# SamGalanakis/FlowCompare

Hardware: AMD Instinct MI355X
Metric: nats/sec (forward log-prob) on 4096-pt coloured pairs (higher is better)
Workload: dtype fp16x2 split (fp32-equivalent operands, f32 accumulate) / f32; 1 GPU; c2_dgcnn_attn_spline: batch 16 scenes/GPU x 4096 target + 4096 context points, 115 flow layers (RationalQuadraticSplineCoupling), embedder DGCNNembedder; global_batch=16, parallelism=scene-sharded x1, no data-path collective

## Files before the change

### flowcompare_amd/csrc/mlprows.hip

```cpp
#include "common.h"
#include "activations.h"
#include "mlprows.h"
#include <type_traits>
#include <cstdio>

namespace fc {

typedef float floatx16 __attribute__((ext_vector_type(16)));
typedef _Float16 f16x8 __attribute__((ext_vector_type(8)));
typedef __attribute__((address_space(3))) char mr_lds_char;
typedef const __attribute__((address_space(1))) char mr_glb_char;

constexpr int MR_KSTG = 8;
constexpr int MR_STAGE = MR_KSTG * 2 * 1024;
constexpr int MR_R = 8, MR_D = 6;
constexpr int MR_PPW = MR_KSTG * 2 / 4;
constexpr int MR_NWAIT = (MR_D - 1) * MR_PPW;
constexpr int MR_BIAS_OFF = MR_R * MR_STAGE;
constexpr int MR_LDS = MR_BIAS_OFF + 2 * MR_HID * 4;

__device__ __forceinline__ void mr_swap32(unsigned& a, unsigned& b) {
    asm("s_nop 1\n\tv_permlane32_swap_b32 %0, %1\n\ts_nop 1" : "+v"(a), "+v"(b));
}
__device__ __forceinline__ unsigned mr_pack(_Float16 a, _Float16 b) {
    return (unsigned)__builtin_bit_cast(unsigned short, a) | ((unsigned)__builtin_bit_cast(unsigned short, b) << 16);
}
__device__ __forceinline__ float mr_lo(unsigned w) { return (float)__builtin_bit_cast(_Float16, (unsigned short)(w & 0xffffu)); }
__device__ __forceinline__ float mr_hi(unsigned w) { return (float)__builtin_bit_cast(_Float16, (unsigned short)(w >> 16)); }

typedef unsigned mr_u4 __attribute__((ext_vector_type(4)));
typedef float mr_f4 __attribute__((ext_vector_type(4)));
__device__ __forceinline__ mr_u4 mr_gload16(const char* ptr) {
    mr_u4 r;
    asm volatile("global_load_dwordx4 %0, %1, off" : "=v"(r) : "v"(ptr) : "memory");
    return r;
}
template <int N>
__device__ __forceinline__ void mr_wait_vm(mr_u4& a, mr_u4& b) {
    asm volatile("s_waitcnt vmcnt(%2)" : "+v"(a), "+v"(b) : "n"(N) : "memory");
}
__device__ __forceinline__ mr_f4 mr_lds_read16(unsigned addr) {
    mr_f4 r;
    asm volatile("ds_read_b128 %0, %1" : "=v"(r) : "v"(addr) : "memory");
    return r;
}
__device__ __forceinline__ void mr_wait_lgkm(mr_f4& a, mr_f4& b, mr_f4& c, mr_f4& d) {
    asm volatile("s_waitcnt lgkmcnt(0)" : "+v"(a), "+v"(b), "+v"(c), "+v"(d) : : "memory");
}

template <int ACT>
__device__ __forceinline__ float mr_act(float v) {
    if constexpr (ACT == FC_ACT_GELU) return fc_gelu(v);
    else if constexpr (ACT == FC_ACT_RELU) return v > 0.f ? v : 0.f;
    else if constexpr (ACT == FC_ACT_ELU) return v > 0.f ? v : expm1f(v);
    else if constexpr (ACT == FC_ACT_LRELU02) return v > 0.f ? v : 0.2f * v;
    else return v;
}

#define MR_STAMP(K_)                                                                                                  \
    if (STAMPS && p.stamps && tid == 0 && (blockIdx.x == 0 || blockIdx.x == 300) && gcur < 256) {                               \
        __builtin_amdgcn_sched_barrier(0);                                                                            \
        p.stamps[((blockIdx.x ? 1 : 0) * 256 + (gcur - ((K_) > 2 ? 1 : 0))) * 8 + (K_)] = __builtin_amdgcn_s_memtime(); \
        __builtin_amdgcn_sched_barrier(0);                                                                            \
    }

template <int KS0, int ACT, bool STAMPS = false>
__global__ __launch_bounds__(256) __attribute__((amdgpu_waves_per_eu(1, 1)))
void mlp_rows_kernel(const MlpRowsParams p) {
    extern __shared__ char smc[];
    const int tid = threadIdx.x, lane = tid & 63, li = lane & 31, lh = lane >> 5;
    const int wave = __builtin_amdgcn_readfirstlane(tid >> 6);
    const int row = blockIdx.x * 128 + wave * 32 + li;
    const int row_in = row < p.rows_valid ? row : p.rows_valid - 1;
    const size_t band = (size_t)blockIdx.x * 4 + wave;
    const size_t band_bytes = (size_t)MR_HID / 16 * 2048;

    const char* ws_ptr = reinterpret_cast<const char*>(p.L[0].Wf) + (wave * MR_PPW) * 1024;
    const unsigned lane16 = lane * 16;
    int ws_left = (p.L[0].ks / MR_KSTG) * MR_NB, ws_layer = 0;
    unsigned ws_slot = 0;
    auto issue_piece = [&](auto i_tag) __attribute__((always_inline)) {
        constexpr int i = decltype(i_tag)::value;
        char* dst = smc + ws_slot * MR_STAGE + (wave * MR_PPW + i) * 1024;
        __builtin_amdgcn_global_load_lds((mr_glb_char*)(ws_ptr + i * 1024 + lane16), (mr_lds_char*)dst, 16, 0, 0);
        if constexpr (i == MR_PPW - 1) {
            ws_slot = (ws_slot + 1) % MR_R;
            if (--ws_left > 0) ws_ptr += MR_STAGE;
            else if (ws_layer + 1 < p.nlayers) {
                ++ws_layer;
                ws_ptr = reinterpret_cast<const char*>(p.L[ws_layer].Wf) + (wave * MR_PPW) * 1024;
                ws_left = (p.L[ws_layer].ks / MR_KSTG) * MR_NB;
            } else ws_left = 1;
        }
    };
    auto issue_stage = [&]() __attribute__((always_inline)) {
        issue_piece(std::integral_constant<int, 0>{}); issue_piece(std::integral_constant<int, 1>{});
        issue_piece(std::integral_constant<int, 2>{}); issue_piece(std::integral_constant<int, 3>{});
    };
    static_assert(MR_PPW == 4, "issue_stage / the slot table place four DMA pieces per wave and stage");
    auto stage_bias = [&](int l) __attribute__((always_inline)) {
        const MlpRowsLayer& L = p.L[l];
        if (wave < 2)
            __builtin_amdgcn_global_load_lds((mr_glb_char*)(reinterpret_cast<const char*>(L.bias) + wave * 1024 + lane * 16),
                                             (mr_lds_char*)(smc + MR_BIAS_OFF + wave * 1024), 16, 0, 0);
        else if (l == 0) {
            if (p.rowscal && L.colvec)
                __builtin_amdgcn_global_load_lds((mr_glb_char*)(reinterpret_cast<const char*>(L.colvec) + (wave - 2) * 1024 + lane * 16),
                                                 (mr_lds_char*)(smc + MR_BIAS_OFF + MR_HID * 4 + (wave - 2) * 1024), 16, 0, 0);
            else
                *reinterpret_cast<float4*>(smc + MR_BIAS_OFF + MR_HID * 4 + (wave - 2) * 1024 + lane * 16) = make_float4(0.f, 0.f, 0.f, 0.f);
        }
    };
    stage_bias(0);
#pragma unroll
    for (int i = 0; i < MR_D; ++i) issue_stage();
    unsigned gcur = 0;

    f16x8 xin[MR_HID / 16][2];
    float omax = 0.f;
    constexpr int MR_XA = 24;
    auto pin_xin = [&](int ks) __attribute__((always_inline)) {
#pragma unroll
        for (int s = 0; s < MR_HID / 16; ++s)
            if (s < MR_XA && s < ks) { asm volatile("" : "+a"(xin[s][0])); asm volatile("" : "+a"(xin[s][1])); }
    };

    {
        const int k0 = p.segk[0], k1 = k0 + p.segk[1], k2 = k1 + p.segk[2];
        float4 raw[KS0][2];
#pragma unroll
        for (int s = 0; s < KS0; ++s) {
            const int seg = s < k0 ? 0 : (s < k1 ? 1 : 2);
            const int sl = s - (seg == 0 ? 0 : (seg == 1 ? k0 : k1));
            const bool live = s < k2;
            const float* ptr = p.A[live ? seg : 0] + (size_t)row_in * p.lda[live ? seg : 0] + (live ? sl : 0) * 16 + 8 * lh;
            raw[s][0] = *reinterpret_cast<const float4*>(ptr);
            raw[s][1] = *reinterpret_cast<const float4*>(ptr + 4);
            if (!live) { raw[s][0] = make_float4(0.f, 0.f, 0.f, 0.f); raw[s][1] = raw[s][0]; }
        }
#pragma unroll
        for (int s = 0; s < KS0; ++s) {
            const float x[8] = {raw[s][0].x, raw[s][0].y, raw[s][0].z, raw[s][0].w, raw[s][1].x, raw[s][1].y, raw[s][1].z, raw[s][1].w};
#pragma unroll
            for (int e = 0; e < 8; ++e) {
                omax = fmaxf(omax, fabsf(x[e]));
                const _Float16 h = (_Float16)x[e];
                xin[s][0][e] = h;
                xin[s][1][e] = (_Float16)((x[e] - (float)h) * 2048.0f);
            }
        }
    }

    pin_xin(KS0);

    floatx16 accA, corrA, accB, corrB;
    mr_u4 resA_hi, resA_lo, resB_hi, resB_lo;
    mr_f4 bnext[4], cnext[4];
    unsigned outq[4][2][2];

    auto run_layer = [&](auto ks_tag, auto res_tag, auto first_tag, const int l) __attribute__((always_inline)) {
        constexpr int KS = decltype(ks_tag)::value;
        constexpr bool HAS_RES = decltype(res_tag)::value;
        constexpr bool FIRST = decltype(first_tag)::value;
        constexpr int NSB = KS / MR_KSTG;
        static_assert(!HAS_RES || NSB == 4, "only the 512 -> 512 hidden layers carry a residual");
        const MlpRowsLayer& L = p.L[l];
        const bool last = l + 1 == p.nlayers;
        const float sp1 = last ? p.out_s1 : 1.0f, sp2 = last ? p.out_s2 : 2048.0f;
        const char* resbase = HAS_RES ? reinterpret_cast<const char*>(p.hbuf[L.res]) + band * band_bytes + lane * 16 : nullptr;
        char* outbase = last ? reinterpret_cast<char*>(p.out16) + (size_t)row * (MR_HID / 16 * 64) + lh * 16
                             : reinterpret_cast<char*>(p.hbuf[L.out]) + band * band_bytes + lane * 16;
        const int out_ss = last ? 64 : 2048, out_ls = last ? 32 : 1024;
        const float rs = (FIRST && p.rowscal && L.colvec) ? p.rowscal[row_in] : 0.f;
        const unsigned bias_lds = (unsigned)(uintptr_t)(mr_lds_char*)smc + (unsigned)(MR_BIAS_OFF + 16 * lh);

        auto bias_fetch = [&](int nb) __attribute__((always_inline)) {
#pragma unroll
            for (int g = 0; g < 4; ++g) {
                bnext[g] = mr_lds_read16(bias_lds + (unsigned)(nb * 32 + 8 * g) * 4u);
                if constexpr (FIRST) cnext[g] = mr_lds_read16(bias_lds + (unsigned)(MR_HID + nb * 32 + 8 * g) * 4u);
            }
        };
        auto init_vec = [&]() __attribute__((always_inline)) -> floatx16 {
            mr_wait_lgkm(bnext[0], bnext[1], bnext[2], bnext[3]);
            if constexpr (FIRST) mr_wait_lgkm(cnext[0], cnext[1], cnext[2], cnext[3]);
            floatx16 b;
#pragma unroll
            for (int g = 0; g < 4; ++g)
#pragma unroll
                for (int t = 0; t < 4; ++t) {
                    b[4 * g + t] = bnext[g][t];
                    if constexpr (FIRST) b[4 * g + t] += rs * cnext[g][t];
                }
            return b;
        };

        float ev[2][4], eu[2][4], eg[2][4];
        auto epi_step = [&](const floatx16& pa, const floatx16& pc, auto g_tag, auto m_tag) __attribute__((always_inline)) {
            constexpr int g = decltype(g_tag)::value, m = decltype(m_tag)::value, pr = m / 12, hs = m % 12, Q = g & 1;
            static_assert(ACT == FC_ACT_GELU, "the interleaved epilogue is written for the exact-erf GELU of the shipped configurations");
            constexpr float C[12] = {7.953413483363647e-10f, -3.609737220244824e-08f, 7.156736501201522e-07f, -8.034509846766014e-06f, 5.399647488957271e-05f, -0.0001862359931692481f, -0.0002285758382640779f, 0.00727660721167922f, -0.05270823836326599f, -0.4591129422187805f, -1.151120901107788f, -0.9999995827674866f};
#define MR_PIN(X_) asm volatile("" : "+v"(X_))
#pragma unroll
            for (int tt = 0; tt < 2; ++tt) {
                const int t = 2 * pr + tt;
                if constexpr (hs == 0) {
                    float v = fmaf(pc[4 * g + t], 1.0f / 2048.0f, pa[4 * g + t]);
                    if constexpr (HAS_RES) {
                        const mr_u4& rh = g < 2 ? resA_hi : resB_hi;
                        const mr_u4& rl = g < 2 ? resA_lo : resB_lo;
                        const unsigned hw = (g & 1) ? (pr == 0 ? rh.z : rh.w) : (pr == 0 ? rh.x : rh.y);
                        const unsigned lw = (g & 1) ? (pr == 0 ? rl.z : rl.w) : (pr == 0 ? rl.x : rl.y);
                        v += tt ? limb_join<1>(hw, lw) : limb_join<0>(hw, lw);
                    }
                    MR_PIN(v);
                    ev[Q][t] = v;
                } else if constexpr (hs == 1) {
                    float u = fminf(fabsf(ev[Q][t]), 7.353910524340095f);
                    float gp = fmaf(C[0], u, C[1]);
                    MR_PIN(u); MR_PIN(gp);
                    eu[Q][t] = u; eg[Q][t] = gp;
                } else if constexpr (hs >= 2 && hs <= 4) {
                    float gp = eg[Q][t];
#pragma unroll
                    for (int c = 0; c < 3; ++c) gp = fmaf(gp, eu[Q][t], C[3 * hs - 4 + c]);
                    MR_PIN(gp);
                    eg[Q][t] = gp;
                } else if constexpr (hs == 5) {
                    float gp = fmaf(eg[Q][t], eu[Q][t], C[11]);
                    MR_PIN(gp);
                    eg[Q][t] = gp;
                } else if constexpr (hs == 6) {
                    float e = __builtin_amdgcn_exp2f(eg[Q][t]);
                    MR_PIN(e);
                    eg[Q][t] = e;
                } else if constexpr (hs == 7) {
                    float m;
                    asm("v_max_f32 %0, 0, %1" : "=v"(m) : "v"(ev[Q][t]));
                    float r = fmaf(-fabsf(ev[Q][t]), eg[Q][t], m);
                    MR_PIN(r);
                    ev[Q][t] = r;
                } else if constexpr (hs == 8) {
                    if (tt == 1) {
                        unsigned wh2, wl2;
                        limb_split2s(ev[Q][2 * pr], ev[Q][2 * pr + 1], sp1, sp2, wh2, wl2);
                        MR_PIN(wh2); MR_PIN(wl2);
                        outq[g][0][pr] = wh2;
                        outq[g][1][pr] = wl2;
                    }
                } else if constexpr (hs == 9) {
                    if (tt == 1) {
                        float om = fmaxf(omax, fmaxf(fabsf(ev[Q][2 * pr]), fabsf(ev[Q][2 * pr + 1])));
                        MR_PIN(om);
                        omax = om;
                    }
                }
            }
#undef MR_PIN
        };
        auto quarter = [&](const floatx16& pa, const floatx16& pc, auto g_tag) __attribute__((always_inline)) {
            auto go = [&](auto... ms) __attribute__((always_inline)) { (epi_step(pa, pc, g_tag, ms), ...); };
            go(std::integral_constant<int, 0>{}, std::integral_constant<int, 1>{}, std::integral_constant<int, 2>{}, std::integral_constant<int, 3>{},
               std::integral_constant<int, 4>{}, std::integral_constant<int, 5>{}, std::integral_constant<int, 6>{}, std::integral_constant<int, 7>{},
               std::integral_constant<int, 8>{}, std::integral_constant<int, 9>{}, std::integral_constant<int, 10>{}, std::integral_constant<int, 11>{},
               std::integral_constant<int, 12>{}, std::integral_constant<int, 13>{}, std::integral_constant<int, 14>{}, std::integral_constant<int, 15>{},
               std::integral_constant<int, 16>{}, std::integral_constant<int, 17>{}, std::integral_constant<int, 18>{}, std::integral_constant<int, 19>{},
               std::integral_constant<int, 20>{}, std::integral_constant<int, 21>{}, std::integral_constant<int, 22>{}, std::integral_constant<int, 23>{});
        };
        auto flush_pair = [&](int fb, auto h_tag) __attribute__((always_inline)) {
            constexpr int h = decltype(h_tag)::value, g = 2 * h + 1;
#pragma unroll
            for (int limb = 0; limb < 2; ++limb) {
                mr_swap32(outq[g - 1][limb][0], outq[g][limb][0]);
                mr_swap32(outq[g - 1][limb][1], outq[g][limb][1]);
                const uint4 frag = make_uint4(outq[g - 1][limb][0], outq[g - 1][limb][1], outq[g][limb][0], outq[g][limb][1]);
                *reinterpret_cast<uint4*>(outbase + (2 * fb + h) * out_ss + limb * out_ls) = frag;
            }
        };
        auto flush_limb = [&](int fb, auto h_tag, auto limb_tag) __attribute__((always_inline)) {
            constexpr int h = decltype(h_tag)::value, g = 2 * h + 1, limb = decltype(limb_tag)::value;
            mr_swap32(outq[g - 1][limb][0], outq[g][limb][0]);
            mr_swap32(outq[g - 1][limb][1], outq[g][limb][1]);
            const uint4 frag = make_uint4(outq[g - 1][limb][0], outq[g - 1][limb][1], outq[g][limb][0], outq[g][limb][1]);
            *reinterpret_cast<uint4*>(outbase + (2 * fb + h) * out_ss + limb * out_ls) = frag;
        };
        auto res_load = [&](int rb, int h, mr_u4& rh, mr_u4& rl) __attribute__((always_inline)) {
            const char* src = resbase + (size_t)((2 * rb + h) * 2) * 1024;
            rh = mr_gload16(src);
            rl = mr_gload16(src + 1024);
        };
        auto res_fix = [&](mr_u4& rh, mr_u4& rl) __attribute__((always_inline)) {
            unsigned a0 = rh.x, a1 = rh.y, a2 = rh.z, a3 = rh.w, b0 = rl.x, b1 = rl.y, b2 = rl.z, b3 = rl.w;
            mr_swap32(a0, a2); mr_swap32(a1, a3);
            mr_swap32(b0, b2); mr_swap32(b1, b3);
            rh.x = a0; rh.y = a1; rh.z = a2; rh.w = a3; rl.x = b0; rl.y = b1; rl.z = b2; rl.w = b3;
        };

        auto block = [&](floatx16& acc, floatx16& corr, const floatx16& pa, const floatx16& pc, const int nb) __attribute__((always_inline)) {
            const int pb = nb > 0 ? nb - 1 : 0;
            const floatx16 binit = init_vec();
            const floatx16 zero16 = {0.f, 0.f, 0.f, 0.f, 0.f, 0.f, 0.f, 0.f, 0.f, 0.f, 0.f, 0.f, 0.f, 0.f, 0.f, 0.f};
            auto stage = [&](auto q_tag) __attribute__((always_inline)) {
                constexpr int q = decltype(q_tag)::value;
                MR_STAMP(0)
                if ((gcur & 1u) == 0u) {
                    asm volatile("s_waitcnt vmcnt(%0)" ::"n"(MR_NWAIT - MR_PPW) : "memory");
                    MR_STAMP(1)
                    __builtin_amdgcn_s_barrier();
                }
                MR_STAMP(2)
                const char* sb = smc + (gcur % MR_R) * MR_STAGE + lane * 16;
                ++gcur;
                __builtin_amdgcn_sched_barrier(0);
                constexpr int QA = NSB == 4 ? q : (NSB == 2 ? 2 * q : (q == 0 ? 0 : q + 1));
                constexpr int QN = NSB == 4 ? 1 : (NSB == 2 ? 2 : (q == 0 ? 2 : 1));
                constexpr int FLUSH_A = NSB == 4 ? 2 : 1;
                f16x8 wh[2], wl[2];
                wh[0] = *reinterpret_cast<const f16x8*>(sb);
                wl[0] = *reinterpret_cast<const f16x8*>(sb + 1024);
                auto slot = [&](auto i_tag) __attribute__((always_inline)) {
                    constexpr int i = decltype(i_tag)::value;
                    if constexpr (i % 6 == 1) issue_piece(std::integral_constant<int, i / 6>{});
                    if constexpr (i == 2 && q == NSB - 1) bias_fetch(nb + 1 < MR_NB ? nb + 1 : nb);
                    if constexpr (NSB == 4 && HAS_RES) {
                        if constexpr (i == 3 && q == 0) res_load(pb, 1, resB_hi, resB_lo);
                        if constexpr (i == 3 && q == 2) res_load(nb, 0, resA_hi, resA_lo);
                        if constexpr (i == 23 && q == 1) { mr_wait_vm<6>(resB_hi, resB_lo); res_fix(resB_hi, resB_lo); }
                        if constexpr (i == 23 && q == 3) { mr_wait_vm<6>(resA_hi, resA_lo); res_fix(resA_hi, resA_lo); }
                    }
                    if constexpr (q == 0 && (i == 4 || i == 5))
                        flush_limb(nb > 1 ? nb - 2 : 0, std::integral_constant<int, 1>{}, std::integral_constant<int, i - 4>{});
                    if constexpr (q == FLUSH_A && (i == 4 || i == 5))
                        flush_limb(pb, std::integral_constant<int, 0>{}, std::integral_constant<int, i - 4>{});
                    epi_step(pa, pc, std::integral_constant<int, QA>{}, i_tag);
                    if constexpr (QN == 2) epi_step(pa, pc, std::integral_constant<int, QA + 1>{}, i_tag);
                    __builtin_amdgcn_sched_barrier(0);
                };
                auto kstep = [&](auto j_tag) __attribute__((always_inline)) {
                    constexpr int j = decltype(j_tag)::value, cur = j & 1, nxt = cur ^ 1, sx = q * MR_KSTG + j;
                    if constexpr (sx == 0) acc = __builtin_amdgcn_mfma_f32_32x32x16_f16(wh[cur], xin[sx][0], binit, 0, 0, 0);
                    else acc = __builtin_amdgcn_mfma_f32_32x32x16_f16(wh[cur], xin[sx][0], acc, 0, 0, 0);
                    if constexpr (j + 1 < MR_KSTG) {
                        wh[nxt] = *reinterpret_cast<const f16x8*>(sb + (2 * j + 2) * 1024);
                        wl[nxt] = *reinterpret_cast<const f16x8*>(sb + (2 * j + 3) * 1024);
                    }
                    slot(std::integral_constant<int, 3 * j>{});
                    if constexpr (sx == 0) corr = __builtin_amdgcn_mfma_f32_32x32x16_f16(wl[cur], xin[sx][0], zero16, 0, 0, 0);
                    else corr = __builtin_amdgcn_mfma_f32_32x32x16_f16(wl[cur], xin[sx][0], corr, 0, 0, 0);
                    slot(std::integral_constant<int, 3 * j + 1>{});
                    corr = __builtin_amdgcn_mfma_f32_32x32x16_f16(wh[cur], xin[sx][1], corr, 0, 0, 0);
                    slot(std::integral_constant<int, 3 * j + 2>{});
                };
                kstep(std::integral_constant<int, 0>{}); kstep(std::integral_constant<int, 1>{}); kstep(std::integral_constant<int, 2>{});
                kstep(std::integral_constant<int, 3>{}); kstep(std::integral_constant<int, 4>{}); kstep(std::integral_constant<int, 5>{});
                kstep(std::integral_constant<int, 6>{}); kstep(std::integral_constant<int, 7>{});
                MR_STAMP(5)
            };
            stage(std::integral_constant<int, 0>{});
            stage(std::integral_constant<int, 1>{});
            if constexpr (NSB > 2) stage(std::integral_constant<int, 2>{});
            if constexpr (NSB > 3) stage(std::integral_constant<int, 3>{});
        };

#pragma unroll
        for (int r = 0; r < 16; ++r) { accB[r] = 0.f; corrB[r] = 0.f; }
        if constexpr (HAS_RES) { res_load(0, 0, resA_hi, resA_lo); mr_wait_vm<0>(resA_hi, resA_lo); }
        asm volatile("s_waitcnt vmcnt(0) lgkmcnt(0)" ::: "memory");
        __builtin_amdgcn_s_barrier();
        bias_fetch(0);
        for (int nb = 0; nb < MR_NB; nb += 2) {
            block(accA, corrA, accB, corrB, nb);
            block(accB, corrB, accA, corrA, nb + 1);
        }
        if constexpr (HAS_RES) {
            res_load(MR_NB - 1, 0, resA_hi, resA_lo);
            res_load(MR_NB - 1, 1, resB_hi, resB_lo);
            mr_wait_vm<0>(resA_hi, resA_lo);
            mr_wait_vm<0>(resB_hi, resB_lo);
            res_fix(resA_hi, resA_lo);
            res_fix(resB_hi, resB_lo);
        }
        flush_pair(MR_NB - 2, std::integral_constant<int, 1>{});
        quarter(accB, corrB, std::integral_constant<int, 0>{});
        quarter(accB, corrB, std::integral_constant<int, 1>{});
        flush_pair(MR_NB - 1, std::integral_constant<int, 0>{});
        quarter(accB, corrB, std::integral_constant<int, 2>{});
        quarter(accB, corrB, std::integral_constant<int, 3>{});
        flush_pair(MR_NB - 1, std::integral_constant<int, 1>{});
    };

    run_layer(std::integral_constant<int, KS0>{}, std::false_type{}, std::true_type{}, 0);
    for (int l = 1; l < p.nlayers; ++l) {
        asm volatile("s_waitcnt vmcnt(0) lgkmcnt(0)" ::: "memory");
        __builtin_amdgcn_s_barrier();
        stage_bias(l);
        const char* src = reinterpret_cast<const char*>(p.hbuf[p.L[l].in]) + band * band_bytes + lane * 16;
#pragma unroll
        for (int s = 0; s < MR_HID / 16; ++s) {
            xin[s][0] = *reinterpret_cast<const f16x8*>(src + (size_t)(2 * s) * 1024);
            xin[s][1] = *reinterpret_cast<const f16x8*>(src + (size_t)(2 * s + 1) * 1024);
        }
        pin_xin(MR_HID / 16);
        if (p.L[l].res >= 0) run_layer(std::integral_constant<int, MR_HID / 16>{}, std::true_type{}, std::false_type{}, l);
        else run_layer(std::integral_constant<int, MR_HID / 16>{}, std::false_type{}, std::false_type{}, l);
    }
    asm volatile("s_waitcnt vmcnt(0)" ::: "memory");
    if (!(omax < p.range_limit) && p.ovf) atomicOr(p.ovf, 1);
}

__global__ __launch_bounds__(256) void mr_frag_image_kernel(const unsigned short* __restrict__ W2, int ks_src, int ks_dst, uint4* __restrict__ Wf, long n16) {
    const long i = (long)blockIdx.x * 256 + threadIdx.x;
    if (i >= n16) return;
    const int lane = (int)(i & 63);
    const long f = i >> 6;
    const int limb = (int)(f & 1);
    const long bs = f >> 1;
    const int s = (int)(bs % ks_dst);
    const long nb = bs / ks_dst;
    uint4 v = make_uint4(0u, 0u, 0u, 0u);
    if (s < ks_src) v = *reinterpret_cast<const uint4*>(W2 + (((size_t)(nb * 32 + (lane & 31)) * ks_src + s) * 2 + limb) * 16 + 8 * (lane >> 5));
    Wf[i] = v;
}

int mlp_rows_ks_pad(int K_pad) {
    const int ks = K_pad / 16;
    return ks <= 16 ? 16 : (ks <= 24 ? 24 : 32);
}
size_t mlp_rows_image_bytes(int K_pad) { return (size_t)MR_NB * mlp_rows_ks_pad(K_pad) * 2048; }

void launch_mlp_rows_image(const PackedLinear& L, unsigned short* Wf, hipStream_t s) {
    if (!L.W2 || L.N_pad != MR_HID || L.K_pad % 16 != 0 || L.K_pad > MR_HID || L.n_alloc < MR_HID)
        throw Error(FC_ERR_INVALID, "launch_mlp_rows_image: layer is not a K <= 512 -> 512 layer with an fp16 limb image");
    const int ksd = mlp_rows_ks_pad(L.K_pad);
    const long n16 = (long)MR_NB * ksd * 2 * 64;
    mr_frag_image_kernel<<<dim3((unsigned)((n16 + 255) / 256)), dim3(256), 0, s>>>(L.W2, L.K_pad / 16, ksd, reinterpret_cast<uint4*>(Wf), n16);
    FC_HIP(hipGetLastError());
}

__global__ __launch_bounds__(256) void mr_limb_decode_kernel(const unsigned short* __restrict__ img, float* __restrict__ out, int ldo, long n, int width) {
    const long i = (long)blockIdx.x * 256 + threadIdx.x;
    if (i >= n) return;
    const long r = i / width;
    const int c = (int)(i - r * width);
    const unsigned short* q = img + ((size_t)r * (width / 16) + (c >> 4)) * 32 + (c & 15);
    out[(size_t)r * ldo + c] = (float)__builtin_bit_cast(_Float16, q[0]) + (float)__builtin_bit_cast(_Float16, q[16]) * (1.0f / 2048.0f);
}
void launch_limb_decode(const unsigned short* img, float* out, int ldo, int rows, int width, hipStream_t s) {
    const long n = (long)rows * width;
    if (n <= 0) return;
    mr_limb_decode_kernel<<<dim3((unsigned)((n + 255) / 256)), dim3(256), 0, s>>>(img, out, ldo, n, width);
    FC_HIP(hipGetLastError());
}

extern int g_gemm_stamp;
unsigned long long* gemm_stamp_buffer(size_t n);
int g_mlp_rows = 1;

template <int KS0, int ACT, bool STAMPS = false>
static void mr_launch(const MlpRowsParams& p, int rows_alloc, double flops, hipStream_t s) {
    auto kern = mlp_rows_kernel<KS0, ACT, STAMPS>;
    static PerDeviceOnce attr_once;
    attr_once.run([&](int) { FC_HIP(hipFuncSetAttribute(reinterpret_cast<const void*>(kern), hipFuncAttributeMaxDynamicSharedMemorySize, MR_LDS)); return 0; });
    char name[96];
    snprintf(name, sizeof name, "void fc::mlp_rows_kernel<%d, %d, %s>(fc::MlpRowsParams)", KS0, ACT, STAMPS ? "true" : "false");
    ProfScope ps(name, flops, 0.0, s);
    hipLaunchKernelGGL(kern, dim3(rows_alloc / 128), dim3(256), MR_LDS, s, p);
    FC_HIP(hipGetLastError());
}

bool mlp_rows_fills_the_chip(int rows_alloc) {
    static PerDeviceOnce cus_once;
    const int cus = cus_once.run([](int dev) {
        int n = 0;
        FC_HIP(hipDeviceGetAttribute(&n, hipDeviceAttributeMultiprocessorCount, dev));
        return n;
    });
    return g_mlp_rows == 2 || rows_alloc / 128 >= (3 * cus) / 4;
}

bool mlp_rows_eligible(const PackedLinear& in, const std::vector<PackedLinear>& mid, int act) {
    if (!g_mlp_rows || act != FC_ACT_GELU) return false;
    if (!in.Wf || in.N_pad != MR_HID || in.K_pad > MR_HID || in.nseg < 1 || in.nseg > 3 || !in.bias) return false;
    for (int i = 0; i < in.nseg; ++i) if (in.seg_k[i] % 16 != 0) return false;
    if (mid.empty() || (int)mid.size() + 1 > MR_MAXL) return false;
    for (const PackedLinear& L : mid) if (!L.Wf || L.N_pad != MR_HID || L.K_pad != MR_HID || L.nseg != 1 || !L.bias) return false;
    return true;
}

void launch_mlp_rows(const PackedLinear& in, const std::vector<PackedLinear>& mid, const ASeg* segs, const float* rowscal, int act,
                     float* const h[3], unsigned short* out16, int rows_alloc, int rows_valid, hipStream_t s, float out16_scale) {
    if (!mlp_rows_eligible(in, mid, act)) throw Error(FC_ERR_UNSUPPORTED, "launch_mlp_rows: shapes outside the row-resident chain");
    if (rows_alloc % 128 != 0 || !out16) throw Error(FC_ERR_INVALID, "launch_mlp_rows: rows must be padded to 128 and a limb-image output given");
    int* flag = gemm_fp16_flag();
    if (!flag) throw Error(FC_ERR_INVALID, "launch_mlp_rows: needs an open split-fp16 guard scope");
    MlpRowsParams p{};
    for (int i = 0; i < 3; ++i) {
        p.A[i] = i < in.nseg ? segs[i].ptr : segs[0].ptr;
        p.lda[i] = i < in.nseg ? segs[i].lda : segs[0].lda;
        p.segk[i] = i < in.nseg ? in.seg_k[i] / 16 : 0;
        if (i < in.nseg && (segs[i].lda % 4 != 0 || ((uintptr_t)segs[i].ptr & 15) || segs[i].lda < in.seg_k[i]))
            throw Error(FC_ERR_INVALID, "launch_mlp_rows: A segment must be 16-byte aligned and at least as wide as its k range");
    }
    p.rowscal = rowscal;
    p.nlayers = 1 + (int)mid.size();
    p.ovf = flag;
    p.out16 = out16;
    p.out_s1 = out16_scale > 0.f ? out16_scale : 1.0f;
    p.out_s2 = out16_scale > 0.f ? 1.0f : 2048.0f;
    p.range_limit = 65504.0f / p.out_s1;
    p.rows_valid = rows_valid > 0 ? rows_valid : rows_alloc;
    for (int i = 0; i < 3; ++i) p.hbuf[i] = reinterpret_cast<unsigned short*>(h[i]);
    const int ks0 = mlp_rows_ks_pad(in.K_pad);
    p.L[0] = MlpRowsLayer{in.Wf, in.bias, in.colvec, ks0, -1, -1, 0};
    int cur = 0, keep = -1;
    double macs = (double)(in.k_true ? in.k_true : in.K_pad) * (in.n_true ? in.n_true : in.N_pad);
    for (size_t i = 0; i < mid.size(); ++i) {
        if (i % 2 == 0) keep = cur;
        int nxt = 0;
        while (nxt == cur || nxt == keep) ++nxt;
        p.L[i + 1] = MlpRowsLayer{mid[i].Wf, mid[i].bias, nullptr, MR_HID / 16, (i % 2 == 1) ? keep : -1, cur, nxt};
        macs += (double)(mid[i].k_true ? mid[i].k_true : mid[i].K_pad) * (mid[i].n_true ? mid[i].n_true : mid[i].N_pad);
        cur = nxt;
    }
    if (g_gemm_stamp == 4) {
        p.stamps = gemm_stamp_buffer(2 * 256 * 8);
        FC_HIP(hipMemsetAsync(p.stamps, 0, 2 * 256 * 8 * sizeof(unsigned long long), s));
    }
    const double flops = 2.0 * (double)(rows_valid > 0 ? rows_valid : rows_alloc) * macs;
    if (ks0 == 16 && p.stamps) mr_launch<16, FC_ACT_GELU, true>(p, rows_alloc, flops, s);
    else if (ks0 == 16) mr_launch<16, FC_ACT_GELU>(p, rows_alloc, flops, s);
    else if (ks0 == 24) mr_launch<24, FC_ACT_GELU>(p, rows_alloc, flops, s);
    else mr_launch<32, FC_ACT_GELU>(p, rows_alloc, flops, s);
}

}
```

Baseline: 393,700 nats/sec.

## Overlap next-layer activation and bias loads with current layer's epilogue

Splits each MLP layer into block, handover and finish phases. During the handover, the next layer's input rows are prefetched from the hidden buffer, the next bias goes into a double-buffered LDS slot, and the last output fragments are kept in registers instead of being re-read. This removes the full vmcnt/lgkmcnt drain and barrier between layers, and it drops the early residual load. In exchange, synchronisation becomes more intricate: the code waits on partial vmcnt values (62, 4), and reading rows written by other waves now relies on a single barrier placed after those partial waits.

```diff
diff --git a/flowcompare_amd/csrc/mlprows.hip b/flowcompare_amd/csrc/mlprows.hip
--- a/flowcompare_amd/csrc/mlprows.hip
+++ b/flowcompare_amd/csrc/mlprows.hip
@@ -17,7 +17,8 @@
 constexpr int MR_PPW = MR_KSTG * 2 / 4;
 constexpr int MR_NWAIT = (MR_D - 1) * MR_PPW;
 constexpr int MR_BIAS_OFF = MR_R * MR_STAGE;
-constexpr int MR_LDS = MR_BIAS_OFF + 2 * MR_HID * 4;
+constexpr int MR_COL_OFF = MR_BIAS_OFF + 2 * MR_HID * 4;
+constexpr int MR_LDS = MR_COL_OFF + MR_HID * 4;
 
 __device__ __forceinline__ void mr_swap32(unsigned& a, unsigned& b) {
     asm("s_nop 1\n\tv_permlane32_swap_b32 %0, %1\n\ts_nop 1" : "+v"(a), "+v"(b));
@@ -98,20 +99,20 @@
         issue_piece(std::integral_constant<int, 2>{}); issue_piece(std::integral_constant<int, 3>{});
     };
     static_assert(MR_PPW == 4, "issue_stage / the slot table place four DMA pieces per wave and stage");
-    auto stage_bias = [&](int l) __attribute__((always_inline)) {
-        const MlpRowsLayer& L = p.L[l];
+    auto stage_bias = [&]() __attribute__((always_inline)) {
+        const MlpRowsLayer& L = p.L[0];
         if (wave < 2)
             __builtin_amdgcn_global_load_lds((mr_glb_char*)(reinterpret_cast<const char*>(L.bias) + wave * 1024 + lane * 16),
                                              (mr_lds_char*)(smc + MR_BIAS_OFF + wave * 1024), 16, 0, 0);
-        else if (l == 0) {
+        else {
             if (p.rowscal && L.colvec)
                 __builtin_amdgcn_global_load_lds((mr_glb_char*)(reinterpret_cast<const char*>(L.colvec) + (wave - 2) * 1024 + lane * 16),
-                                                 (mr_lds_char*)(smc + MR_BIAS_OFF + MR_HID * 4 + (wave - 2) * 1024), 16, 0, 0);
+                                                 (mr_lds_char*)(smc + MR_COL_OFF + (wave - 2) * 1024), 16, 0, 0);
             else
-                *reinterpret_cast<float4*>(smc + MR_BIAS_OFF + MR_HID * 4 + (wave - 2) * 1024 + lane * 16) = make_float4(0.f, 0.f, 0.f, 0.f);
-        }
-    };
-    stage_bias(0);
+                *reinterpret_cast<float4*>(smc + MR_COL_OFF + (wave - 2) * 1024 + lane * 16) = make_float4(0.f, 0.f, 0.f, 0.f);
+        }
+    };
+    stage_bias();
 #pragma unroll
     for (int i = 0; i < MR_D; ++i) issue_stage();
     unsigned gcur = 0;
@@ -123,6 +124,21 @@
 #pragma unroll
         for (int s = 0; s < MR_HID / 16; ++s)
             if (s < MR_XA && s < ks) { asm volatile("" : "+a"(xin[s][0])); asm volatile("" : "+a"(xin[s][1])); }
+    };
+
+    auto xload = [&](const char* base, auto s_tag) __attribute__((always_inline)) {
+        constexpr int S = decltype(s_tag)::value;
+        const char* sb = base + S * 2048 + lane16;
+        xin[S][0] = *reinterpret_cast<const f16x8*>(sb);
+        xin[S][1] = *reinterpret_cast<const f16x8*>(sb + 1024);
+    };
+    auto xin_ready = [&](const int s0, const int s1) __attribute__((always_inline)) {
+#pragma unroll
+        for (int s = 0; s < MR_HID / 16; ++s)
+            if (s >= s0 && s < s1) {
+                if (s < MR_XA) { asm volatile("" : "+a"(xin[s][0])); asm volatile("" : "+a"(xin[s][1])); }
+                else { asm volatile("" : "+v"(xin[s][0])); asm volatile("" : "+v"(xin[s][1])); }
+            }
     };
 
     {
@@ -158,8 +174,8 @@
     mr_f4 bnext[4], cnext[4];
     unsigned outq[4][2][2];
 
-    auto run_layer = [&](auto ks_tag, auto res_tag, auto first_tag, const int l) __attribute__((always_inline)) {
-        constexpr int KS = decltype(ks_tag)::value;
+    auto run_layer = [&](auto ks_tag, auto res_tag, auto first_tag, const int l, auto part_tag) __attribute__((always_inline)) {
+        constexpr int KS = decltype(ks_tag)::value, PART = decltype(part_tag)::value;
         constexpr bool HAS_RES = decltype(res_tag)::value;
         constexpr bool FIRST = decltype(first_tag)::value;
         constexpr int NSB = KS / MR_KSTG;
@@ -172,13 +188,16 @@
                              : reinterpret_cast<char*>(p.hbuf[L.out]) + band * band_bytes + lane * 16;
         const int out_ss = last ? 64 : 2048, out_ls = last ? 32 : 1024;
         const float rs = (FIRST && p.rowscal && L.colvec) ? p.rowscal[row_in] : 0.f;
-        const unsigned bias_lds = (unsigned)(uintptr_t)(mr_lds_char*)smc + (unsigned)(MR_BIAS_OFF + 16 * lh);
+        const unsigned bias_lds = (unsigned)(uintptr_t)(mr_lds_char*)smc + (unsigned)(MR_BIAS_OFF + (l & 1) * (MR_HID * 4) + 16 * lh);
+        const char* xnext = reinterpret_cast<const char*>(p.hbuf[L.out]) + band * band_bytes;
+        const char* bias_next = reinterpret_cast<const char*>(p.L[PART == 1 ? l + 1 : l].bias) + wave * 512 + lane * 4;
+        char* bias_next_lds = smc + MR_BIAS_OFF + ((l + 1) & 1) * (MR_HID * 4) + wave * 512;
 
         auto bias_fetch = [&](int nb) __attribute__((always_inline)) {
 #pragma unroll
             for (int g = 0; g < 4; ++g) {
                 bnext[g] = mr_lds_read16(bias_lds + (unsigned)(nb * 32 + 8 * g) * 4u);
-                if constexpr (FIRST) cnext[g] = mr_lds_read16(bias_lds + (unsigned)(MR_HID + nb * 32 + 8 * g) * 4u);
+                if constexpr (FIRST) cnext[g] = mr_lds_read16(bias_lds + (unsigned)(2 * MR_HID + nb * 32 + 8 * g) * 4u);
             }
         };
         auto init_vec = [&]() __attribute__((always_inline)) -> floatx16 {
@@ -267,7 +286,7 @@
                std::integral_constant<int, 16>{}, std::integral_constant<int, 17>{}, std::integral_constant<int, 18>{}, std::integral_constant<int, 19>{},
                std::integral_constant<int, 20>{}, std::integral_constant<int, 21>{}, std::integral_constant<int, 22>{}, std::integral_constant<int, 23>{});
         };
-        auto flush_pair = [&](int fb, auto h_tag) __attribute__((always_inline)) {
+        auto flush_pair = [&](int fb, auto h_tag, auto keep_tag) __attribute__((always_inline)) {
             constexpr int h = decltype(h_tag)::value, g = 2 * h + 1;
 #pragma unroll
             for (int limb = 0; limb < 2; ++limb) {
@@ -275,6 +294,7 @@
                 mr_swap32(outq[g - 1][limb][1], outq[g][limb][1]);
                 const uint4 frag = make_uint4(outq[g - 1][limb][0], outq[g - 1][limb][1], outq[g][limb][0], outq[g][limb][1]);
                 *reinterpret_cast<uint4*>(outbase + (2 * fb + h) * out_ss + limb * out_ls) = frag;
+                if constexpr (decltype(keep_tag)::value) xin[MR_HID / 16 - 2 + h][limb] = __builtin_bit_cast(f16x8, frag);
             }
         };
         auto flush_limb = [&](int fb, auto h_tag, auto limb_tag) __attribute__((always_inline)) {
@@ -362,48 +382,78 @@
             if constexpr (NSB > 3) stage(std::integral_constant<int, 3>{});
         };
 
+        if constexpr (PART == 0) {
 #pragma unroll
         for (int r = 0; r < 16; ++r) { accB[r] = 0.f; corrB[r] = 0.f; }
-        if constexpr (HAS_RES) { res_load(0, 0, resA_hi, resA_lo); mr_wait_vm<0>(resA_hi, resA_lo); }
-        asm volatile("s_waitcnt vmcnt(0) lgkmcnt(0)" ::: "memory");
-        __builtin_amdgcn_s_barrier();
+        if constexpr (HAS_RES) { resA_hi = mr_u4{0u, 0u, 0u, 0u}; resA_lo = resA_hi; }
+        if constexpr (FIRST) {
+            asm volatile("s_waitcnt vmcnt(0) lgkmcnt(0)" ::: "memory");
+            __builtin_amdgcn_s_barrier();
+        }
         bias_fetch(0);
         for (int nb = 0; nb < MR_NB; nb += 2) {
             block(accA, corrA, accB, corrB, nb);
             block(accB, corrB, accA, corrA, nb + 1);
         }
-        if constexpr (HAS_RES) {
-            res_load(MR_NB - 1, 0, resA_hi, resA_lo);
-            res_load(MR_NB - 1, 1, resB_hi, resB_lo);
-            mr_wait_vm<0>(resA_hi, resA_lo);
-            mr_wait_vm<0>(resB_hi, resB_lo);
-            res_fix(resA_hi, resA_lo);
-            res_fix(resB_hi, resB_lo);
-        }
-        flush_pair(MR_NB - 2, std::integral_constant<int, 1>{});
+        } else if constexpr (PART == 2) {
+            if constexpr (HAS_RES) res_load(MR_NB - 1, 1, resB_hi, resB_lo);
+            flush_pair(MR_NB - 2, std::integral_constant<int, 1>{}, std::false_type{});
+            quarter(accB, corrB, std::integral_constant<int, 0>{});
+            quarter(accB, corrB, std::integral_constant<int, 1>{});
+            flush_pair(MR_NB - 1, std::integral_constant<int, 0>{}, std::false_type{});
+            if constexpr (HAS_RES) { mr_wait_vm<4>(resB_hi, resB_lo); res_fix(resB_hi, resB_lo); }
+            quarter(accB, corrB, std::integral_constant<int, 2>{});
+            quarter(accB, corrB, std::integral_constant<int, 3>{});
+            flush_pair(MR_NB - 1, std::integral_constant<int, 1>{}, std::false_type{});
+        } else {
+        {
+            __builtin_amdgcn_global_load_lds((mr_glb_char*)bias_next, (mr_lds_char*)bias_next_lds, 4, 0, 0);
+            __builtin_amdgcn_global_load_lds((mr_glb_char*)(bias_next + 256), (mr_lds_char*)(bias_next_lds + 256), 4, 0, 0);
+            xload(xnext, std::integral_constant<int, 0>{});
+            if constexpr (HAS_RES) res_load(MR_NB - 1, 1, resB_hi, resB_lo);
+            auto go = [&](auto... ss) __attribute__((always_inline)) { (xload(xnext, ss), ...); };
+            go(std::integral_constant<int, 1>{}, std::integral_constant<int, 2>{}, std::integral_constant<int, 3>{}, std::integral_constant<int, 4>{},
+               std::integral_constant<int, 5>{}, std::integral_constant<int, 6>{}, std::integral_constant<int, 7>{}, std::integral_constant<int, 8>{},
+               std::integral_constant<int, 9>{}, std::integral_constant<int, 10>{}, std::integral_constant<int, 11>{}, std::integral_constant<int, 12>{},
+               std::integral_constant<int, 13>{}, std::integral_constant<int, 14>{}, std::integral_constant<int, 15>{}, std::integral_constant<int, 16>{},
+               std::integral_constant<int, 17>{}, std::integral_constant<int, 18>{}, std::integral_constant<int, 19>{}, std::integral_constant<int, 20>{},
+               std::integral_constant<int, 21>{}, std::integral_constant<int, 22>{}, std::integral_constant<int, 23>{}, std::integral_constant<int, 24>{},
+               std::integral_constant<int, 25>{}, std::integral_constant<int, 26>{}, std::integral_constant<int, 27>{}, std::integral_constant<int, 28>{});
+        }
+        flush_pair(MR_NB - 2, std::integral_constant<int, 1>{}, std::false_type{});
+        xload(xnext, std::integral_constant<int, 29>{});
         quarter(accB, corrB, std::integral_constant<int, 0>{});
         quarter(accB, corrB, std::integral_constant<int, 1>{});
-        flush_pair(MR_NB - 1, std::integral_constant<int, 0>{});
+        flush_pair(MR_NB - 1, std::integral_constant<int, 0>{}, std::true_type{});
+        if constexpr (HAS_RES) { mr_wait_vm<62>(resB_hi, resB_lo); res_fix(resB_hi, resB_lo); }
         quarter(accB, corrB, std::integral_constant<int, 2>{});
         quarter(accB, corrB, std::integral_constant<int, 3>{});
-        flush_pair(MR_NB - 1, std::integral_constant<int, 1>{});
-    };
-
-    run_layer(std::integral_constant<int, KS0>{}, std::false_type{}, std::true_type{}, 0);
+        flush_pair(MR_NB - 1, std::integral_constant<int, 1>{}, std::true_type{});
+        asm volatile("s_waitcnt vmcnt(4)" ::: "memory");
+        xin_ready(0, MR_HID / 16);
+        __builtin_amdgcn_s_barrier();
+        }
+    };
+
+    constexpr std::integral_constant<int, MR_HID / 16> KSH{};
+    constexpr std::integral_constant<int, 0> BLOCKS{};
+    constexpr std::integral_constant<int, 1> HANDOVER{};
+    constexpr std::integral_constant<int, 2> FINISH{};
+    run_layer(std::integral_constant<int, KS0>{}, std::false_type{}, std::true_type{}, 0, BLOCKS);
     for (int l = 1; l < p.nlayers; ++l) {
-        asm volatile("s_waitcnt vmcnt(0) lgkmcnt(0)" ::: "memory");
-        __builtin_amdgcn_s_barrier();
-        stage_bias(l);
-        const char* src = reinterpret_cast<const char*>(p.hbuf[p.L[l].in]) + band * band_bytes + lane * 16;
-#pragma unroll
-        for (int s = 0; s < MR_HID / 16; ++s) {
-            xin[s][0] = *reinterpret_cast<const f16x8*>(src + (size_t)(2 * s) * 1024);
-            xin[s][1] = *reinterpret_cast<const f16x8*>(src + (size_t)(2 * s + 1) * 1024);
-        }
-        pin_xin(MR_HID / 16);
-        if (p.L[l].res >= 0) run_layer(std::integral_constant<int, MR_HID / 16>{}, std::true_type{}, std::false_type{}, l);
-        else run_layer(std::integral_constant<int, MR_HID / 16>{}, std::false_type{}, std::false_type{}, l);
+        if (p.L[l].res >= 0) {
+            run_layer(KSH, std::false_type{}, std::false_type{}, l - 1, HANDOVER);
+            run_layer(KSH, std::true_type{}, std::false_type{}, l, BLOCKS);
+        } else if (p.L[l - 1].res >= 0) {
+            run_layer(KSH, std::true_type{}, std::false_type{}, l - 1, HANDOVER);
+            run_layer(KSH, std::false_type{}, std::false_type{}, l, BLOCKS);
+        } else {
+            run_layer(KSH, std::false_type{}, std::false_type{}, l - 1, HANDOVER);
+            run_layer(KSH, std::false_type{}, std::false_type{}, l, BLOCKS);
+        }
     }
+    if (p.L[p.nlayers - 1].res >= 0) run_layer(KSH, std::true_type{}, std::false_type{}, p.nlayers - 1, FINISH);
+    else run_layer(KSH, std::false_type{}, std::false_type{}, p.nlayers - 1, FINISH);
     asm volatile("s_waitcnt vmcnt(0)" ::: "memory");
     if (!(omax < p.range_limit) && p.ovf) atomicOr(p.ovf, 1);
 }
```

New measurement: 393,400 nats/sec. Within noise of the previous version (-0.1%).
